# jswu18/projected-langevin-sampling

Measured on AMD Instinct MI355X. Metric: Langevin steps/sec, higher is better.
Workload: dtype f64; 1 GPU; configs[1]: synthetic regression N=1e5 M=1024 J=8192 D=8, RBF/ARD, ONB + Gaussian/identity, fp64; N=100000, M=1024, M_k=1024, J=8192, J_per_gpu=8192, parallelism=J-sharded x1, no per-step collective

## Files before the change

projected-langevin-sampling_amd/csrc/plship.hip:

```cpp
#include <hip/hip_runtime.h>

#include <atomic>
#include <cmath>
#include <cstdarg>
#include <cstdio>
#include <cstdlib>
#include <string>
#include <vector>

#define PLS_SCALAR_POLY_CONSTANTS 1
#include "../../include/plship.h"
#include "chol.h"
#include "common.h"
#include "cost_device.h"
#include "gemm_api.h"
#include "gemm_tn_f64.h"
#include "gemm_launch.h"
#include "gemm_tn_f64_kg.h"
#include "gemm_tn_f64_rows.h"
#include "cost_epilogues.h"
#include "philox.h"
#include "small_rank.h"
#include "small_rank_launch.h"
#include "small_rank_step.h"
// ... 2039 lines not shown

static int validate_onb(const pls_onb_desc *b) {
  PLS_REQUIRE(b != nullptr, "onb descriptor is NULL");
  PLS_REQUIRE(b->mk > 0 && b->n > 0, "onb: mk and n must be positive");
  PLS_REQUIRE(b->A && b->At && b->lam, "onb: A, At and lam must be set");
  PLS_REQUIRE(b->lda >= b->n && b->ldat >= b->mk, "onb: leading dimension too small");
  if (b->B) PLS_REQUIRE(b->ldb >= b->mk && b->c, "onb: B needs ldb >= mk and c");
  return PLS_OK;
}

int pls_onb_build_projection(const double *Vs, int64_t ldvs, const double *Kzx, int64_t ldkzx, int64_t m, int64_t mk,
                             int64_t n, double *A, int64_t lda, double *At, int64_t ldat, void *stream) {
  PLS_REQUIRE(Vs && Kzx && A && At, "onb_build_projection: NULL pointer");
  PLS_REQUIRE(m > 0 && mk > 0 && n > 0 && mk <= m, "onb_build_projection: bad sizes");
  PLS_REQUIRE(ldvs >= mk && ldkzx >= n && lda >= n && ldat >= mk, "onb_build_projection: leading dimension too small");
  int rc = pls_gemm_tn(Vs, ldvs, Kzx, ldkzx, A, lda, mk, n, m, 1.0, 0.0, stream);
  if (rc) return rc;
  return pls_gemm_tn(Kzx, ldkzx, Vs, ldvs, At, ldat, n, mk, m, 1.0, 0.0, stream);
}

int pls_onb_build_gaussian(const pls_onb_desc *basis, const double *y, double *B, int64_t ldb, double *c, void *stream) {
  int rc = validate_onb(basis);
  if (rc) return rc;
  PLS_REQUIRE(y && B && c && ldb >= basis->mk, "onb_build_gaussian: bad arguments");
  rc = pls_gemm_tn(basis->At, basis->ldat, basis->At, basis->ldat, B, ldb, basis->mk, basis->mk, basis->n, 1.0, 0.0, stream);
  if (rc) return rc;
  hipLaunchKernelGGL(matvec_rows_kernel, dim3((unsigned)basis->mk), dim3(256), 0, S(stream), basis->A, basis->lda,
                     basis->n, y, c);
  rc = check_launch("matvec_rows");
  if (rc) return rc;
  hipLaunchKernelGGL(matvec_rows_kernel, dim3(1), dim3(256), 0, S(stream), y, basis->n, basis->n, y, c + basis->mk);
  return check_launch("matvec_rows");
}

int pls_onb_forward(const pls_onb_desc *basis, const double *U, int64_t ldu, int64_t j, double *F, int64_t ldf,
                    void *stream) {
  int rc = validate_onb(basis);
  if (rc) return rc;
  PLS_REQUIRE(U && F && j >= 0 && ldu >= j && ldf >= j, "onb_forward: bad arguments");
  return pls_gemm_tn(basis->A, basis->lda, U, ldu, F, ldf, basis->n, j, basis->mk, 1.0, 0.0, stream);
}

int pls_onb_particle_update(const pls_onb_desc *basis, const double *U, int64_t ldu, const double *G, int64_t ldg,
                            int64_t j, double eta, const pls_noise_desc *noise, double *dU, int64_t lddu, void *stream) {
  int rc = validate_onb(basis);
  if (rc) return rc;
  rc = validate_noise(noise, j);
  if (rc) return rc;
  PLS_REQUIRE(U && G && dU && j >= 0 && ldu >= j && ldg >= j && lddu >= j, "onb_particle_update: bad arguments");
  PLS_REQUIRE(eta >= 0.0, "onb_particle_update: step size must be >= 0");
  if (j == 0) return PLS_OK;
  rc = pls_gemm_tn(basis->At, basis->ldat, G, ldg, dU, lddu, basis->mk, j, basis->n, 1.0, 0.0, stream);
  if (rc) return rc;
  hipLaunchKernelGGL(langevin_update_kernel, dim3((unsigned)cdiv(j, 256), rows_grid(cdiv(basis->mk, 8) * 4)), dim3(256), 0,
                     S(stream), dU, lddu, U, ldu, dU, lddu, 1, (int64_t)0, U, ldu, basis->lam, 0.0, basis->mk, j,
                     make_etap(eta, nullptr), 0, make_noisep(noise));
  return check_launch("langevin_update");
}


struct StepCall {
  const pls_cost_desc *cost;
  const double *y;
  const double *U;
  int64_t ldu, j;
  double eta;
  const pls_block_desc *blocks;
  const pls_noise_desc *noise;
  double *out;
  int64_t ldo;
  int32_t out_mode;
  double *energy_in;
  void *workspace;
  size_t workspace_bytes;
  hipStream_t st;
  EtaP etap() const { return make_etap(eta, blocks); }
  NoiseP noisep() const { return make_noisep(noise, blocks); }
  double *energy_sums() const { return blocks ? blocks->energy_sums : nullptr; }
  uint32_t *energy_sync() const { return blocks ? blocks->energy_sync : nullptr; }
};

static int validate_blocks(const pls_block_desc *b) {
  if (!b) return PLS_OK;
  PLS_REQUIRE(b->block_cols > 0 && b->eta != nullptr, "step_blocks: block_cols must be > 0 and eta set");
  return PLS_OK;
}

static int validate_step(const char *who, const StepCall &c, bool lagged) {
  if (int rc = validate_cost(c.cost)) return rc;
  if (int rc = validate_noise(c.noise, c.j)) return rc;
  if (int rc = validate_blocks(c.blocks)) return rc;
  if (lagged) return validate_lag(c.blocks);
  PLS_REQUIRE(!c.blocks || (!c.blocks->energy_partials && !c.blocks->energy_partials_prev && !c.blocks->energy_flush),
              "%s: lagged energies (energy_partials) exist on the Gaussian/identity routes only", who);
  return PLS_OK;
}

static int validate_step_call(const char *who, const StepCall &c, bool needs_y) {
  PLS_REQUIRE(c.U && c.out && (c.y || !needs_y), "%s: NULL pointer", who);
  PLS_REQUIRE(c.out != c.U, "%s: out must not alias the particles (ping-pong the particle buffers)", who);
  PLS_REQUIRE(c.j >= 0 && c.ldu >= c.j && c.ldo >= c.j, "%s: bad sizes", who);
  PLS_REQUIRE(c.eta >= 0.0, "%s: step size must be >= 0", who);
  PLS_REQUIRE(c.out_mode == 0 || c.out_mode == 1, "%s: out_mode must be 0 (delta) or 1 (new state)", who);
  return PLS_OK;
}

enum class StepRoute { Whitened, Fast, OneLaunch, General, Winograd };

static bool gaussian_fast_path(const double *B, const double *c, const pls_cost_desc *cost, int force_generic) {
  return !force_generic && B && c && cost->cost == PLS_COST_GAUSSIAN && cost->link == PLS_LINK_IDENTITY;
}

static bool ws_holds(size_t total, const void *workspace, size_t workspace_bytes) {
  return total == 0 || (workspace && total <= workspace_bytes);
}

static bool launch_bound(int64_t n, int64_t mk, int64_t j) { return j <= 4096 && 4.0 * (double)n * (double)mk * (double)j <= 8e9; }

static bool sr_step_route_for(const double *Lb, int64_t ldlb, int64_t mk, int64_t n, const double *y, int64_t j) {
  const int64_t mode = g_small_rank_step.load();
  if (mode == 0 || !small_rank_ok(Lb, ldlb, mk)) return false;
  if (reinterpret_cast<uintptr_t>(y) & 15) return false;
  return mode >= 2 || launch_bound(n, mk, j);
}

struct SrStepOperands {
  const double *Lb;
  int64_t ldlb, mk, n;
  const double *Vf;
  int64_t ldvf;
  const double *Uadd;
  int64_t lduadd;
  const double *lam;
  double pconst;
  int64_t n_data = -1;
};

static SrStepLayout sr_step_plan(int lead, int64_t mk, int64_t n, const StepCall &c) {
  return sr_step_layout(lead, mk, n, c.j, c.blocks && c.energy_in && c.blocks->energy_sums, c.blocks && c.blocks->step_sync);
}

static int sr_step_launch(const SrStepOperands &basis, const SrStepLayout &L, const StepCall &c, const NoiseP &nz) {
  char *w = static_cast<char *>(c.workspace);
  uint32_t *sync = c.blocks ? c.blocks->step_sync : nullptr;
  if (L.counters) {
    sync = reinterpret_cast<uint32_t *>(w + L.sync_off);
    hipError_t e = hipMemsetAsync(sync, 0, L.sync_bytes, c.st);
    if (e != hipSuccess) return fail(PLS_ERR_HIP, "onb_step: hipMemsetAsync: %s", hipGetErrorString(e));
  }
  const int64_t ncb = cdiv(c.j, 16);
  SrStepP p{};
  p.Lb = basis.Lb;
  p.ldlb = basis.ldlb;
  p.U = basis.Vf;
  p.ldu = basis.ldvf;
  p.Uadd = basis.Uadd;
  p.lduadd = basis.lduadd;
  p.y = c.y;
  p.lam = basis.lam;
  p.pconst = basis.pconst;
  p.N = basis.n;
  p.Ndata = basis.n_data >= 0 ? basis.n_data : basis.n;
  p.J = c.j;
  p.K = (int)basis.mk;
  p.rows_per_split = L.rows;
  p.nsplit = (int)L.ns;
  p.cp = make_costp(c.cost);
  p.out = c.out;
  p.ldo = c.ldo;
  p.add_u = c.out_mode;
  p.etap = c.etap();
  p.nz = nz;
  p.cb_sync = sync;
  p.chunk_sync = sync ? sync + ncb : nullptr;
  p.slab = reinterpret_cast<double *>(w + L.slab_off);
  p.vslab = p.slab ? p.slab + ncb * L.ns * basis.mk * 16 : nullptr;
  p.e = c.energy_in;
  p.esums = (c.blocks && c.energy_in) ? c.blocks->energy_sums : nullptr;
  p.sums16 = (c.blocks && c.energy_in) ? c.blocks->energy_sums16 : nullptr;
#ifdef PLS_SRS_PROBE
  p.debug_stop = getenv("PLS_SRS_STOP") ? atoi(getenv("PLS_SRS_STOP")) : 0;
#endif
  if (p.Ndata < p.N) return c.energy_in ? launch_small_rank_step_prior_value(p, c.st) : launch_small_rank_step_prior(p, c.st);
  return c.energy_in ? launch_small_rank_step_value(p, c.st) : launch_small_rank_step(p, c.st);
}

static int finish_energy_sums(const pls_block_desc *blocks, const double *energy_in, int64_t j, hipStream_t st) {
  if (!blocks || !energy_in) return PLS_OK;
  if (blocks->energy_sums) {
    hipLaunchKernelGGL(chunk_sums_kernel, dim3((unsigned)cdiv(j, 256)), dim3(256), 0, st, energy_in, j, blocks->energy_sums);
    if (int rc = check_launch("chunk_sums")) return rc;
  }
  if (blocks->energy_sums16) {
    hipLaunchKernelGGL(sums16_kernel, dim3((unsigned)cdiv(cdiv(j, 16), 256)), dim3(256), 0, st, energy_in, j, blocks->energy_sums16);
    if (int rc = check_launch("sums16")) return rc;
  }
  return PLS_OK;
}

static int finish_sums16(const pls_block_desc *blocks, const double *energy_in, int64_t j, hipStream_t st) {
  if (!blocks || !energy_in || !blocks->energy_sums16 || blocks->energy_partials) return PLS_OK;
  hipLaunchKernelGGL(sums16_kernel, dim3((unsigned)cdiv(cdiv(j, 16), 256)), dim3(256), 0, st, energy_in, j, blocks->energy_sums16);
  return check_launch("sums16");
}

static int fast_step(const FastOp &op, const StepCall &c, const char *who) {
  const int rc = fast_step_launch(op, c.U, c.ldu, c.j, c.etap(), c.noisep(), c.out, c.ldo, c.out_mode, c.energy_in, c.workspace,
                                  c.workspace_bytes, c.st, who, c.energy_sums(), c.energy_sync(), make_lag(c.blocks));
  return rc ? rc : finish_sums16(c.blocks, c.energy_in, c.j, c.st);
}


static FastOp onb_fast_op(const pls_onb_desc *b, const pls_cost_desc *c) {
  return FastOp{b->B, b->ldb, b->c, b->lam, b->mk, 1.0 / c->p[0], 0.5 / c->p[0], b->c + b->mk};
}

static bool wino_basis_ok(const pls_onb_desc *b) {
  auto al = [](const void *p, int64_t ld) { return (reinterpret_cast<uintptr_t>(p) & 15) == 0 && (ld & 1) == 0; };
  return b->mk % 16 == 0 && b->mk >= 512 && b->n % 4 == 0 && b->n >= 16384 && al(b->A, b->lda) && al(b->At, b->ldat);
}

constexpr int64_t kWinoMinChunk = 8192;

static bool wino_route_for(const pls_onb_desc *b, const double *planes, size_t planes_bytes, const double *U, int64_t ldu,
                           int64_t j) {
  return g_winograd.load() != 0 && planes && (reinterpret_cast<uintptr_t>(planes) & 15) == 0 && wino_basis_ok(b) &&
         planes_bytes >= 4 * wino_left_plane_bytes(b->mk, b->n) && j % 128 == 0 && j >= 2048 &&
         (reinterpret_cast<uintptr_t>(U) & 15) == 0 && (ldu & 1) == 0;
}

size_t pls_onb_winograd_bytes(const pls_onb_desc *basis) {
  return (basis && validate_onb(basis) == PLS_OK && wino_basis_ok(basis)) ? 4 * wino_left_plane_bytes(basis->mk, basis->n) : 0;
}

int pls_onb_winograd_prepare(const pls_onb_desc *basis, double *planes, size_t planes_bytes, void *stream) {
  int rc = validate_onb(basis);
  if (rc) return rc;
  PLS_REQUIRE(wino_basis_ok(basis), "onb_winograd_prepare: the basis' shape or operands do not take the Winograd route");
  const size_t plane = wino_left_plane_bytes(basis->mk, basis->n);
  PLS_REQUIRE(planes && (reinterpret_cast<uintptr_t>(planes) & 15) == 0 && planes_bytes >= 4 * plane,
              "onb_winograd_prepare: planes must be 16-byte aligned and hold %zu bytes", 4 * plane);
  const int64_t mh = basis->mk / 2, nh = basis->n / 2;
  {
    LaunchScope scope(PLS_TAG_OTHER, S(stream));
    hipLaunchKernelGGL(winograd_left_kernel, dim3((unsigned)cdiv(mh, 256), (unsigned)(nh < 8192 ? nh : 8192)), dim3(256), 0,
                       S(stream), basis->At, basis->ldat, nh, mh, planes, (int64_t)(plane / sizeof(double)));
  }
  return check_launch("winograd_left");
}

size_t pls_onb_step_workspace_bytes(const pls_onb_desc *basis, int64_t j, int64_t n_chunk) {
  if (!basis || j <= 0) return 0;
  if (n_chunk <= 0 || n_chunk > basis->n) n_chunk = basis->n;
  const size_t general = drift_layout(0, basis->mk, basis->n, j, n_chunk).total;
  const size_t one_launch = sr_step_query_bytes(0, basis->mk, basis->n, j);
  return general > one_launch ? general : one_launch;
}

static int onb_general_step(const pls_onb_desc *basis, const StepCall &c) {
  const DriftLayout L = drift_plan(0, basis->mk, basis->n, c.j, c.workspace_bytes);
  if (!c.workspace || L.total > c.workspace_bytes)
    return fail(PLS_ERR_WORKSPACE_TOO_SMALL, "onb_step: workspace %zu bytes, need at least %zu", c.workspace_bytes,
                pls_onb_step_workspace_bytes(basis, c.j, 128));
  char *w = static_cast<char *>(c.workspace);
  double *D = reinterpret_cast<double *>(w + L.d_off);
  const int64_t slab_stride = (int64_t)(L.mj / sizeof(double));
  EnergySink sink;
  if (c.energy_in) {
    sink.partial = reinterpret_cast<double *>(w + L.part_off);
    sink.rows_cap = L.part_rows;
    sink.e = c.energy_in;
    sink.prior_kind = 1;
    sink.P = c.U;
    sink.ldp = c.ldu;
    sink.m = basis->mk;
    sink.lam = basis->lam;
  }
  int64_t nslab = 1;
  int rc = stream_drift(basis->A, basis->lda, basis->At, basis->ldat, basis->mk, basis->n, c.U, c.ldu, c.j, make_costp(c.cost),
                        c.y, D, c.j, L.slabs, slab_stride, &nslab, reinterpret_cast<double *>(w + L.g_off), L.n_chunk, c.st,
                        c.energy_in ? &sink : nullptr);
  if (rc) return rc;
  {
    LaunchScope scope(PLS_TAG_LANGEVIN_UPDATE, c.st);
    hipLaunchKernelGGL(langevin_update_kernel, dim3((unsigned)cdiv(c.j, 256), rows_grid(cdiv(basis->mk, 8) * 4)), dim3(256), 0,
                       c.st, c.out, c.ldo, c.U, c.ldu, D, c.j, (int)nslab, slab_stride, c.U, c.ldu, basis->lam, 0.0, basis->mk,
                       c.j, c.etap(), c.out_mode, c.noisep());
  }
  rc = check_launch("langevin_update");
  if (rc) return rc;
  return finish_energy_sums(c.blocks, c.energy_in, c.j, c.st);
}

static int onb_wino_step(const pls_onb_desc *basis, const StepCall &c, const WinoLayout &L, const double *S) {
  char *w = static_cast<char *>(c.workspace);
  double *P = reinterpret_cast<double *>(w + L.p_off);
  double *Q = reinterpret_cast<double *>(w + L.q_off);
  double *part = reinterpret_cast<double *>(w + L.part_off);
  const int64_t mh = L.mh, nh = L.nh, jh = L.jh, mk = basis->mk;
  const int64_t splane = (int64_t)(L.s_plane / sizeof(double)), pslab = (int64_t)(L.p_slab / sizeof(double));
  const int64_t qplane = (int64_t)(L.q_plane / sizeof(double));
  int rc = PLS_OK;
  int64_t kchunk = 0;
  const int64_t nslab = wino_split_k(mh, jh, L.n_chunk, &kchunk);
  const CostP cp = make_costp(c.cost);
  const double *At = basis->At;
  const int64_t ldat = basis->ldat;
  for (int64_t p0 = 0, ci = 0; p0 < nh; p0 += L.n_chunk, ++ci) {
    const int64_t rows = (nh - p0 < L.n_chunk) ? (nh - p0) : L.n_chunk;
    rc = launch_cost_deriv_paired(basis->A + p0, basis->lda, nh, c.U, c.ldu, jh, rows, mk, Q, qplane, c.y + p0, cp,
                                  c.energy_in ? part : nullptr, c.j, c.st);
    if (rc) return rc;
    if (c.energy_in) {
      LaunchScope scope(PLS_TAG_OTHER, c.st);
      hipLaunchKernelGGL(column_reduce_kernel, dim3((unsigned)cdiv(c.j, 256)), dim3(256), 0, c.st, part, c.j, cdiv(rows, 32), c.j,
                         c.energy_in, ci == 0 ? 0 : 1, p0 + L.n_chunk >= nh ? 1 : 0, c.U, c.ldu, mk, basis->lam, 0.0, 1.0,
                         (const double *)nullptr);
      if ((rc = check_launch("column_reduce"))) return rc;
    }
    const double *S1 = S + p0 * mh, *S2 = S1 + splane, *S3 = S2 + splane, *S4 = S3 + splane;
    const double *A11 = At + p0 * ldat, *A12 = At + (nh + p0) * ldat, *A22 = A12 + mh;
    WinoProducts t{{A11, A12, S4, A22, S1, S2, S3},
                   {ldat, ldat, mh, ldat, mh, mh, mh},
                   {Q + WQ_G11 * qplane, Q + WQ_G21 * qplane, Q + WQ_G22 * qplane, Q + WQ_T4 * qplane, Q + WQ_T1 * qplane,
                    Q + WQ_T2 * qplane, Q + WQ_T3 * qplane},
                   nslab * pslab};
    rc = launch_wino_products(t, mh, jh, rows, nslab > 1 ? kchunk : 0, P, pslab, ci == 0 ? 0.0 : 1.0, c.st);
    if (rc) return rc;
  }
  {
    LaunchScope scope(PLS_TAG_LANGEVIN_UPDATE, c.st);
    hipLaunchKernelGGL(langevin_update_wino_kernel, dim3((unsigned)cdiv(jh, 256), rows_grid(cdiv(mh, 8) * 4)), dim3(256), 0, c.st,
                       c.out, c.ldo, c.U, c.ldu, P, (int)nslab, pslab, basis->lam, mh, jh, c.etap(), c.out_mode, c.noisep());
  }
  rc = check_launch("langevin_update_wino");
  if (rc) return rc;
  return finish_energy_sums(c.blocks, c.energy_in, c.j, c.st);
}

static int onb_step_impl(const pls_onb_desc *basis, const StepCall &c, int32_t force_generic, const double *wg_planes = nullptr,
                         size_t wg_bytes = 0) {
  int rc = validate_onb(basis);
  if (!rc) rc = validate_step("onb_step", c, true);
  if (rc) return rc;
  const bool fast = gaussian_fast_path(basis->B, basis->c, c.cost, force_generic);
  if (c.blocks && c.blocks->energy_flush) {
    PLS_REQUIRE(fast, "onb_step: energy_flush is for the Gaussian/identity fast path");
    PLS_REQUIRE(c.U && c.j > 0 && c.ldu >= c.j, "onb_step: energy_flush needs the particle matrix of the step calls");
    return fast_step_launch(onb_fast_op(basis, c.cost), c.U, c.ldu, c.j, c.etap(), c.noisep(), nullptr, 0, 0, nullptr, nullptr, 0,
                            c.st, "onb_step", nullptr, nullptr, make_lag(c.blocks));
  }
  if ((rc = validate_step_call("onb_step", c, true))) return rc;
  if (c.j == 0) return PLS_OK;
  StepRoute route = StepRoute::General;
  SrStepLayout sl{};
  if (fast) {
    route = StepRoute::Fast;
  } else if (sr_step_route_for(basis->At, basis->ldat, basis->mk, basis->n, c.y, c.j)) {
    sl = sr_step_plan(0, basis->mk, basis->n, c);
    if (ws_holds(sl.total, c.workspace, c.workspace_bytes)) route = StepRoute::OneLaunch;
  }
  WinoLayout wl{};
  if (route == StepRoute::General && wino_route_for(basis, wg_planes, wg_bytes, c.U, c.ldu, c.j)) {
    wl = wino_plan(basis->mk, basis->n, c.j, c.workspace_bytes);
    const int64_t min_chunk = wl.nh < kWinoMinChunk ? wl.nh : kWinoMinChunk;
    if (c.workspace && wl.total <= c.workspace_bytes && wl.n_chunk >= min_chunk) route = StepRoute::Winograd;
  }
  PLS_REQUIRE(fast || !c.blocks || (!c.blocks->energy_partials && !c.blocks->energy_partials_prev),
              "onb_step: lagged energies (energy_partials) exist on the Gaussian/identity fast path only");
  switch (route) {
    case StepRoute::Fast:
      return fast_step(onb_fast_op(basis, c.cost), c, "onb_step");
    case StepRoute::OneLaunch:
      return sr_step_launch(SrStepOperands{basis->At, basis->ldat, basis->mk, basis->n, c.U, c.ldu, nullptr, 0, basis->lam, 0.0},
                            sl, c, c.noisep());
    case StepRoute::Winograd:
      return onb_wino_step(basis, c, wl, wg_planes);
    default:
      return onb_general_step(basis, c);
  }
}

int pls_onb_step(const pls_onb_desc *basis, const pls_cost_desc *cost, const double *y, double *U, int64_t ldu,
                 int64_t j, double eta, const pls_noise_desc *noise, double *out, int64_t ldo, int32_t out_mode,
                 int32_t force_generic, double *energy_in, void *workspace, size_t workspace_bytes, void *stream) {
  return onb_step_impl(basis, StepCall{cost, y, U, ldu, j, eta, nullptr, noise, out, ldo, out_mode, energy_in, workspace,
                                       workspace_bytes, S(stream)}, force_generic);
}

int pls_onb_step_wg(const pls_onb_desc *basis, const pls_cost_desc *cost, const double *y, double *U, int64_t ldu, int64_t j,
                    double eta, const pls_noise_desc *noise, double *out, int64_t ldo, int32_t out_mode, int32_t force_generic,
                    const double *wg_planes, size_t wg_bytes, double *energy_in, void *workspace, size_t workspace_bytes,
                    void *stream) {
  return onb_step_impl(basis, StepCall{cost, y, U, ldu, j, eta, nullptr, noise, out, ldo, out_mode, energy_in, workspace,
                                       workspace_bytes, S(stream)}, force_generic, wg_planes, wg_bytes);
}

int pls_onb_step_blocks_wg(const pls_onb_desc *basis, const pls_cost_desc *cost, const double *y, double *U, int64_t ldu,
                           int64_t j, const pls_block_desc *blocks, const pls_noise_desc *noise, double *out, int64_t ldo,
                           int32_t out_mode, int32_t force_generic, const double *wg_planes, size_t wg_bytes, double *energy_in,
                           void *workspace, size_t workspace_bytes, void *stream) {
  PLS_REQUIRE(blocks != nullptr, "onb_step_blocks: block descriptor is NULL");
  return onb_step_impl(basis, StepCall{cost, y, U, ldu, j, 0.0, blocks, noise, out, ldo, out_mode, energy_in, workspace,
                                       workspace_bytes, S(stream)}, force_generic, wg_planes, wg_bytes);
}

int pls_onb_step_blocks(const pls_onb_desc *basis, const pls_cost_desc *cost, const double *y, double *U, int64_t ldu,
                        int64_t j, const pls_block_desc *blocks, const pls_noise_desc *noise, double *out, int64_t ldo,
                        int32_t out_mode, int32_t force_generic, double *energy_in, void *workspace,
                        size_t workspace_bytes, void *stream) {
  PLS_REQUIRE(blocks != nullptr, "onb_step_blocks: block descriptor is NULL");
  return onb_step_impl(basis, StepCall{cost, y, U, ldu, j, 0.0, blocks, noise, out, ldo, out_mode, energy_in, workspace,
                                       workspace_bytes, S(stream)}, force_generic);
}


size_t pls_onb_energy_workspace_bytes(const pls_onb_desc *basis, int64_t j, int64_t n_chunk) {
  if (!basis || j <= 0) return 0;
  if (n_chunk <= 0 || n_chunk > basis->n) n_chunk = basis->n;
  return energy_layout(0, basis->mk, j, n_chunk).total;
}

int pls_onb_energy(const pls_onb_desc *basis, const pls_cost_desc *cost, const double *y, const double *U, int64_t ldu,
                   int64_t j, double *e, int32_t force_generic, void *workspace, size_t workspace_bytes, void *stream) {
  int rc = validate_onb(basis);
  if (rc) return rc;
  rc = validate_cost(cost);
  if (rc) return rc;
  PLS_REQUIRE(U && e && y && j >= 0 && ldu >= j, "onb_energy: bad arguments");
  if (j == 0) return PLS_OK;
  if (gaussian_fast_path(basis->B, basis->c, cost, force_generic))
    return fast_energy_launch(onb_fast_op(basis, cost), U, ldu, j, e, workspace, workspace_bytes, S(stream), "onb_energy");
  const EnergyLayout L = energy_plan(0, basis->mk, basis->n, j, workspace_bytes);
  if (!workspace || L.part_rows < 2)
    return fail(PLS_ERR_WORKSPACE_TOO_SMALL, "onb_energy: workspace %zu bytes too small", workspace_bytes);
  return stream_cost(basis->A, basis->lda, basis->At, basis->ldat, basis->mk, basis->n, U, ldu, j, make_costp(cost), y,
                     reinterpret_cast<double *>(static_cast<char *>(workspace) + L.part_off), L.part_rows, L.n_chunk, e, 1, U,
                     ldu, basis->mk, basis->lam, 0.0, S(stream));
}

int pls_onb_prior_energy(const pls_onb_desc *basis, const double *U, int64_t ldu, int64_t j, const double *cost,
                         double *e, void *stream) {
  int rc = validate_onb(basis);
  if (rc) return rc;
  PLS_REQUIRE(U && e && j >= 0 && ldu >= j, "onb_prior_energy: bad arguments");
  if (j == 0) return PLS_OK;
  hipLaunchKernelGGL(column_reduce_kernel, dim3((unsigned)cdiv(j, 256)), dim3(256), 0, S(stream), cost, j,
                     (int64_t)(cost ? 1 : 0), j, e, 0, 1, U, ldu, basis->mk, basis->lam, 0.0, 1.0, (const double *)nullptr);
  return check_launch("column_reduce");
}


static int validate_ipb(const pls_ipb_desc *b) {
  PLS_REQUIRE(b != nullptr, "ipb descriptor is NULL");
  PLS_REQUIRE(b->m > 0 && b->n > 0, "ipb: m and n must be positive");
  PLS_REQUIRE(b->Kzx && b->Kxz, "ipb: Kzx and Kxz must be set");
  PLS_REQUIRE((b->Sf && b->Sb) || b->W || (b->Linv && b->LinvT),
              "ipb: k(Z,Z) must enter as substitution operators Sf / Sb (pls_chol_factor), as the inverse factor Linv / LinvT or as W");
  PLS_REQUIRE((b->Linv == nullptr) == (b->LinvT == nullptr), "ipb: Linv and LinvT go together");
  if (b->Linv) PLS_REQUIRE(b->ldlinv >= b->m && b->ldlinvt >= b->m, "ipb: ldlinv / ldlinvt < m");
  if (b->Q) PLS_REQUIRE(b->ldq >= b->m && b->ct, "ipb: Q needs ldq >= m and ct");
  PLS_REQUIRE((b->Sf == nullptr) == (b->Sb == nullptr), "ipb: Sf and Sb go together");
  PLS_REQUIRE(b->ldkzx >= b->n && b->ldkxz >= b->m, "ipb: leading dimension too small");
  if (b->W) PLS_REQUIRE(b->ldw >= b->m, "ipb: ldw < m");
  if (b->Sf) PLS_REQUIRE(b->ldsf >= b->m && b->ldsb >= b->m, "ipb: ldsf / ldsb < m");
  if (b->LcT) PLS_REQUIRE(b->ldlct >= b->m, "ipb: ldlct < m");
  if (b->B) PLS_REQUIRE(b->ldb >= b->m && b->c, "ipb: fast-path constants need ldb >= m and c");
  return PLS_OK;
}

static pls_chol_desc ipb_factor(const pls_ipb_desc *b) {
  return pls_chol_desc{b->m, nullptr, 0, b->LcT, b->ldlct, b->Sf, b->ldsf, b->Sb, b->ldsb, b->Linv, b->ldlinv, b->LinvT, b->ldlinvt,
                       b->tri_scratch, b->tri_scratch_bytes};
}

static int ipb_apply_kinv(const pls_ipb_desc *b, const double *U, int64_t ldu, int64_t j, double *V, void *stream,
                          double *tmp = nullptr) {
  const bool explicit_inverse = (!b->Sf && !b->Linv) || (g_ipb_explicit_inverse.load() != 0 && b->W);
  if (explicit_inverse) return pls_gemm_tn(b->W, b->ldw, U, ldu, V, j, b->m, j, b->m, 1.0, 0.0, stream);
  const pls_chol_desc f = ipb_factor(b);
  return chol_full_solve(&f, U, ldu, j, V, j, tmp, S(stream));
}

static bool ipb_whitened_ok(const pls_ipb_desc *b, const pls_cost_desc *c) {
  return b->Q && b->ct && b->LcT && b->ldq >= b->m && b->q_inv_noise == 1.0 / c->p[0] && (b->LinvT || (b->Sf && b->Sb)) &&
         g_ipb_explicit_inverse.load() == 0;
}

static FastOp ipb_whitened_op(const pls_ipb_desc *b) {
  return FastOp{b->Q, b->ldq, b->ct, nullptr, b->m, 1.0, 0.5 * b->q_inv_noise, b->ct + b->m};
}

int pls_ipb_forward(const pls_ipb_desc *basis, const double *U, int64_t ldu, int64_t j, double *F, int64_t ldf,
                    void *workspace, size_t workspace_bytes, void *stream) {
  int rc = validate_ipb(basis);
  if (rc) return rc;
  PLS_REQUIRE(U && F && j >= 0 && ldu >= j && ldf >= j, "ipb_forward: bad arguments");
  if (j == 0) return PLS_OK;
  const size_t need = (size_t)basis->m * j * sizeof(double);
  if (!workspace || workspace_bytes < need)
    return fail(PLS_ERR_WORKSPACE_TOO_SMALL, "ipb_forward: workspace %zu < %zu bytes", workspace_bytes, need);
  double *V = static_cast<double *>(workspace);
  rc = ipb_apply_kinv(basis, U, ldu, j, V, stream);
  if (rc) return rc;
  return pls_gemm_tn(basis->Kzx, basis->ldkzx, V, j, F, ldf, basis->n, j, basis->m, 1.0, 0.0, stream);
}

static int ipb_colour_noise(const pls_ipb_desc *basis, NoiseP &nz, int64_t j, double *xi_buf, double *e_buf, hipStream_t st) {
  if (nz.kind != PLS_NOISE_PHILOX) return PLS_OK;
  if (!basis->LcT) return fail(PLS_ERR_INVALID_ARGUMENT, "ipb: Philox noise needs the Cholesky factor LcT");
  hipLaunchKernelGGL(normal_fill_kernel, dim3((unsigned)cdiv(j, 256), rows_grid(cdiv(basis->m, 8) * 4)), dim3(256), 0, st,
                     xi_buf, j, basis->m, j, nz.seed, nz.step, nz.j_offset, nz.step_base, nz.block_cols);
  int rc = check_launch("normal_fill");
  if (rc) return rc;
  rc = gemm_tn_ex(basis->LcT, basis->ldlct, xi_buf, j, e_buf, j, basis->m, j, basis->m, 1.0, 0.0, 1, st, basis->tri_scratch,
                  basis->tri_scratch_bytes);
  if (rc) return rc;
  nz.kind = PLS_NOISE_INJECTED;
  nz.xi = e_buf;
  nz.ldxi = j;
  return PLS_OK;
}

static int ipb_finish(const pls_ipb_desc *basis, const double *U, int64_t ldu, const double *D, int nslab,
                      int64_t slab_stride, const double *V, int64_t j, double eta, const pls_noise_desc *noise, double *out, int64_t ldo, int add_u,
                      double *xi_buf, double *e_buf, hipStream_t st, const double *dsub = nullptr, double dsub_scale = 0.0,
                      const pls_block_desc *blocks = nullptr) {
  NoiseP nz = make_noisep(noise, blocks);
  if (int rc = ipb_colour_noise(basis, nz, j, xi_buf, e_buf, st)) return rc;
  hipLaunchKernelGGL(langevin_update_kernel, dim3((unsigned)cdiv(j, 256), rows_grid(cdiv(basis->m, 8) * 4)), dim3(256), 0, st,
                     out, ldo, U, ldu, D, j, nslab, slab_stride, V, j, (const double *)nullptr, (double)basis->m, basis->m, j,
                     make_etap(eta, blocks), add_u, nz, dsub, dsub_scale);
  return check_launch("langevin_update");
}

int pls_ipb_build_gaussian(const pls_ipb_desc *basis, const double *y, double *B, int64_t ldb, double *c, void *stream) {
  int rc = validate_ipb(basis);
  if (rc) return rc;
  PLS_REQUIRE(y && B && c && ldb >= basis->m, "ipb_build_gaussian: bad arguments");
  rc = pls_gemm_tn(basis->Kxz, basis->ldkxz, basis->Kxz, basis->ldkxz, B, ldb, basis->m, basis->m, basis->n, 1.0, 0.0, stream);
  if (rc) return rc;
  hipLaunchKernelGGL(matvec_rows_kernel, dim3((unsigned)basis->m), dim3(256), 0, S(stream), basis->Kzx, basis->ldkzx,
                     basis->n, y, c);
  rc = check_launch("matvec_rows");
  if (rc) return rc;
  hipLaunchKernelGGL(matvec_rows_kernel, dim3(1), dim3(256), 0, S(stream), y, basis->n, basis->n, y, c + basis->m);
  return check_launch("matvec_rows");
}

int pls_ipb_particle_update(const pls_ipb_desc *basis, const double *U, int64_t ldu, const double *G, int64_t ldg,
                            int64_t j, double eta, const pls_noise_desc *noise, double *dU, int64_t lddu,
                            void *workspace, size_t workspace_bytes, void *stream) {
  int rc = validate_ipb(basis);
  if (rc) return rc;
  rc = validate_noise(noise, j);
  if (rc) return rc;
  PLS_REQUIRE(U && G && dU && j >= 0 && ldu >= j && ldg >= j && lddu >= j, "ipb_particle_update: bad arguments");
  PLS_REQUIRE(eta >= 0.0, "ipb_particle_update: step size must be >= 0");
  if (j == 0) return PLS_OK;
  const size_t mj = align_up((size_t)basis->m * j * sizeof(double), 256);
  if (!workspace || workspace_bytes < 4 * mj)
    return fail(PLS_ERR_WORKSPACE_TOO_SMALL, "ipb_particle_update: workspace %zu < %zu bytes", workspace_bytes, 4 * mj);
  char *w = static_cast<char *>(workspace);
  double *V = reinterpret_cast<double *>(w), *D = reinterpret_cast<double *>(w + mj);
  double *xi = reinterpret_cast<double *>(w + 2 * mj), *e = reinterpret_cast<double *>(w + 3 * mj);
  rc = ipb_apply_kinv(basis, U, ldu, j, V, stream, xi);
  if (rc) return rc;
  rc = pls_gemm_tn(basis->Kxz, basis->ldkxz, G, ldg, D, j, basis->m, j, basis->n, 1.0, 0.0, stream);
  if (rc) return rc;
  return ipb_finish(basis, U, ldu, D, 1, (int64_t)0, V, j, eta, noise, dU, lddu, 0, xi, e, S(stream));
}

constexpr int IPB_LEAD = 3;

size_t pls_ipb_step_workspace_bytes(const pls_ipb_desc *basis, int64_t j, int64_t n_chunk) {
  if (!basis || j <= 0) return 0;
  if (n_chunk <= 0 || n_chunk > basis->n) n_chunk = basis->n;
  const size_t general = drift_layout(IPB_LEAD, basis->m, basis->n, j, n_chunk).total;
  const size_t one_launch = sr_step_query_bytes(IPB_LEAD, basis->m, basis->n, j);
  return general > one_launch ? general : one_launch;
}

static int ipb_whitened_route(const pls_ipb_desc *basis, const StepCall &c, const DriftLayout &L) {
  char *w = static_cast<char *>(c.workspace);
  double *Sw = reinterpret_cast<double *>(w), *Wd = reinterpret_cast<double *>(w + L.mj);
  double *epart = reinterpret_cast<double *>(w + 2 * L.mj);
  NoiseP nz = c.noisep();
  const bool injected = nz.kind == PLS_NOISE_INJECTED;
  const double *e_inj = injected ? nz.xi : nullptr;
  const int64_t ld_inj = nz.ldxi;
  if (injected) nz.kind = PLS_NOISE_NONE;
  int rc;
  if (basis->Pt && !c.energy_in && g_ipb_step_operator.load() != 0) {
    FastOp op = ipb_whitened_op(basis);
    op.B = basis->Pt;
    op.ldb = basis->ldpt;
    rc = fast_step_launch(op, c.U, c.ldu, c.j, c.etap(), nz, Wd, c.j, 0, nullptr, nullptr, 0, c.st, "ipb_step");
  } else {
    const pls_chol_desc f = ipb_factor(basis);
    rc = chol_forward_solve(&f, c.U, c.ldu, c.j, Sw, c.j, c.st);
    if (rc) return rc;
    rc = fast_step_launch(ipb_whitened_op(basis), Sw, c.j, c.j, c.etap(), nz, Wd, c.j, 0, c.energy_in, epart, 2 * L.mj, c.st,
                          "ipb_step", c.energy_sums(), c.energy_sync());
  }
  if (rc) return rc;
  rc = finish_sums16(c.blocks, c.energy_in, c.j, c.st);
  if (rc) return rc;
  EpiIpbFinish fin{c.out, c.ldo, c.U, c.ldu, c.out_mode, c.etap(), e_inj, ld_inj};
  return launch_gemm_any(basis->LcT, basis->ldlct, Wd, c.j, basis->m, c.j, basis->m, fin, c.st, 0, 1,
                         TriScratch{basis->tri_scratch, basis->tri_scratch_bytes});
}

static int ipb_fast_route(const pls_ipb_desc *basis, const StepCall &c, const DriftLayout &L) {
  char *w = static_cast<char *>(c.workspace);
  double *V = reinterpret_cast<double *>(w), *xi = reinterpret_cast<double *>(w + L.mj);
  double *e = reinterpret_cast<double *>(w + 2 * L.mj), *D = reinterpret_cast<double *>(w + L.d_off);
  int rc = ipb_apply_kinv(basis, c.U, c.ldu, c.j, V, c.st, xi);
  if (rc) return rc;
  const double inv_noise = 1.0 / c.cost->p[0];
// ... 404 lines not shown
```

projected-langevin-sampling_amd/csrc/step_plan.h:

```cpp
#pragma once
#include <cmath>
#include <cstddef>
#include <cstdint>
#ifdef PLS_SRS_PROBE
#include <cstdlib>
#endif

#include "common.h"
#include "small_rank.h"
#include "small_rank_step.h"

namespace plship {

static inline size_t mj_bytes(int64_t m, int64_t j) { return align_up((size_t)m * j * sizeof(double), 256); }

static inline int64_t plan_split_k(int64_t I, int64_t J, int64_t K, int64_t *kchunk) {
  const int64_t tiles = cdiv(I, 128) * cdiv(J, 128);
  int64_t s = 1;
  if (tiles < 512) s = cdiv(512, tiles);
  const int64_t s_local = cdiv(K, 16384);
  if (s_local > s) s = s_local;
  if (s > 16) s = 16;
  if (s > 1) {
    auto waste = [&](int64_t sl) {
      const double rounds = (double)(tiles * sl) / 512.0;
      return std::ceil(rounds) / rounds;
    };
    int64_t best = s;
    for (int64_t sl = s + 1; sl <= 16 && sl <= s + 4; ++sl)
      if (waste(sl) < waste(best) - 0.03) best = sl;
    s = best;
  }
  const int64_t min_chunk = tiles < 64 ? 256 : 1024;
  while (s > 1 && K / s < min_chunk) --s;
  int64_t kc = cdiv(cdiv(K, s), 16) * 16;
  s = cdiv(K, kc);
  *kchunk = (s > 1) ? kc : 0;
  return s;
}

static inline int64_t onb_max_slabs(int64_t mk, int64_t j, int64_t n) {
  int64_t kc;
  int64_t s = plan_split_k(mk, j, n, &kc);
  if (mk <= 256) {
    int64_t rows;
    const int64_t sr = small_rank_splits(j, n, &rows);
    if (sr > s) s = sr;
  }
  return s;
}

static inline int64_t energy_partial_rows(int64_t n_chunk) { return cdiv(n_chunk, 32) < 32 ? 32 : cdiv(n_chunk, 32); }
static inline size_t onb_energy_partial_bytes(int64_t n_chunk, int64_t j) {
  return align_up((size_t)energy_partial_rows(n_chunk) * j * sizeof(double), 256);
}

static inline int64_t gaussian_partial_rows(int64_t mk, bool big_tiles, bool step) {
  return big_tiles ? (step ? 2 : 1) * cdiv(mk, 128) : cdiv(mk, 64);
}
static inline size_t gaussian_partial_bytes(int64_t rows, int64_t j) { return (size_t)rows * j * sizeof(double); }
static inline size_t gaussian_step_partial_bytes(int64_t mk, int64_t j) { return gaussian_partial_bytes(gaussian_partial_rows(mk, true, true), j); }

struct SrStepLayout {
  int64_t ns, rows;
  size_t slab_off, slab_bytes;
  bool counters;
  size_t sync_off, sync_bytes;
  size_t total;
};

static inline SrStepLayout sr_step_layout(int lead, int64_t mk, int64_t n, int64_t j, bool sums, bool own_sync) {
  SrStepLayout L{};
  L.ns = small_rank_step_splits(j, n, (int)mk, &L.rows);
#ifdef PLS_SRS_PROBE
  if (const char *f = getenv("PLS_SRS_FORCE_NS")) {
    L.ns = atoi(f);
    L.rows = (cdiv(n, L.ns) + 63) / 64 * 64;
    L.ns = cdiv(n, L.rows);
  }
#endif
  L.slab_off = (size_t)lead * mj_bytes(mk, j);
  L.slab_bytes = L.ns > 1 ? align_up((size_t)cdiv(j, 16) * L.ns * ((size_t)mk + 1) * 16 * sizeof(double), 256) : 0;
  L.counters = (L.ns > 1 || sums) && !own_sync;
  L.sync_off = L.slab_off + L.slab_bytes;
  L.sync_bytes = small_rank_step_sync_words(j) * sizeof(uint32_t);
  L.total = L.sync_off + (L.counters ? align_up(L.sync_bytes, 256) : 0);
  return L;
}

static inline size_t sr_step_query_bytes(int lead, int64_t mk, int64_t n, int64_t j) {
  return (mk < 1 || mk > 128) ? 0 : sr_step_layout(lead, mk, n, j, true, false).total;
}

struct DriftLayout {
  size_t mj;
  int64_t slabs;
  int64_t n_chunk, part_rows;
  size_t d_off, part_off, g_off, total;
};

static inline DriftLayout drift_chunk(DriftLayout L, int64_t j, int64_t n_chunk) {
  L.n_chunk = n_chunk;
  L.part_rows = energy_partial_rows(n_chunk);
  L.g_off = L.part_off + onb_energy_partial_bytes(n_chunk, j);
  L.total = L.g_off + (size_t)n_chunk * j * sizeof(double);
  return L;
}

static inline DriftLayout drift_layout(int lead, int64_t mk, int64_t n, int64_t j, int64_t n_chunk) {
  DriftLayout L{};
  L.mj = mj_bytes(mk, j);
  L.slabs = onb_max_slabs(mk, j, n);
  L.d_off = (size_t)lead * L.mj;
  L.part_off = L.d_off + (size_t)L.slabs * L.mj;
  return drift_chunk(L, j, n_chunk);
}

static inline DriftLayout drift_plan(int lead, int64_t mk, int64_t n, int64_t j, size_t avail) {
  const DriftLayout all = drift_layout(lead, mk, n, j, n);
  if (all.total <= avail) return all;
  auto fits = [&](int64_t c) { return drift_chunk(all, j, c).total <= avail; };
  const int64_t min_rows = n < 128 ? n : 128;
  if (!fits(min_rows)) return drift_chunk(all, j, min_rows);
  const size_t left = avail - all.part_off;
  const double per_row = (double)j * sizeof(double) * (1.0 + 1.0 / 32.0);
  int64_t c = (int64_t)(((double)left - 32.0 * j * sizeof(double) - 512.0) / per_row);
  if (c > n) c = n;
  c = c / 128 * 128;
  while (c > min_rows && !fits(c)) c -= 128;
  while (c + 128 <= n && fits(c + 128)) c += 128;
  return drift_chunk(all, j, c < min_rows ? min_rows : c);
}

struct WinoLayout {
  int64_t mh, nh, jh;
  int64_t slabs;
  int64_t n_chunk, part_rows;
  size_t s_plane, p_slab, q_plane;
  size_t p_off, part_off, q_off, total;
};

static inline int64_t wino_split_k(int64_t mh, int64_t jh, int64_t K, int64_t *kchunk) {
  const int64_t tiles = 7 * cdiv(mh, 128) * cdiv(jh, 128);
  int64_t s = tiles < 512 ? cdiv(512, tiles) : 1;
  const int64_t s_local = cdiv(K, 16384);
  if (s_local > s) s = s_local;
  if (s > 16) s = 16;
  auto waste = [&](int64_t sl) {
    const double rounds = (double)(tiles * sl) / 512.0;
    return std::ceil(rounds) / rounds;
  };
  int64_t best = s;
  for (int64_t sl = s + 1; sl <= 16 && sl <= s + 4; ++sl)
    if (waste(sl) < waste(best) - 0.03) best = sl;
  s = best;
  while (s > 1 && K / s < 1024) --s;
  int64_t kc = cdiv(cdiv(K, s), 16) * 16;
  s = cdiv(K, kc);
  *kchunk = (s > 1) ? kc : 0;
  return s;
}

static inline size_t wino_left_plane_bytes(int64_t mk, int64_t n) { return align_up((size_t)(n / 2) * (mk / 2) * sizeof(double), 256); }

static inline WinoLayout wino_chunk(WinoLayout L, int64_t n_chunk) {
  L.n_chunk = n_chunk;
  L.part_rows = energy_partial_rows(n_chunk);
  L.q_plane = align_up((size_t)n_chunk * L.jh * sizeof(double), 256);
  L.q_off = L.part_off + align_up((size_t)L.part_rows * 2 * L.jh * sizeof(double), 256);
  L.total = L.q_off + 7 * L.q_plane;
  return L;
}

static inline WinoLayout wino_layout(int64_t mk, int64_t n, int64_t j, int64_t n_chunk) {
  WinoLayout L{};
  L.mh = mk / 2;
  L.nh = n / 2;
  L.jh = j / 2;
  int64_t kc;
  L.slabs = wino_split_k(L.mh, L.jh, n_chunk < L.nh ? n_chunk : L.nh, &kc);
  L.s_plane = wino_left_plane_bytes(mk, n);
  L.p_slab = align_up((size_t)L.mh * L.jh * sizeof(double), 256);
  L.p_off = 0;
  L.part_off = L.p_off + 7 * (size_t)L.slabs * L.p_slab;
  return wino_chunk(L, n_chunk);
}

static inline WinoLayout wino_plan(int64_t mk, int64_t n, int64_t j, size_t avail) {
  const int64_t nh = n / 2;
  const WinoLayout all = wino_layout(mk, n, j, nh);
  if (all.total <= avail) return all;
  const int64_t min_rows = nh < 128 ? nh : 128;
  int64_t c = nh / 128 * 128;
  while (c > min_rows && wino_layout(mk, n, j, c).total > avail) c -= 128;
  return wino_layout(mk, n, j, c < min_rows ? min_rows : c);
}

struct EnergyLayout {
  size_t part_off;
  int64_t part_rows;
  int64_t n_chunk;
  size_t gauss_bytes;
  size_t total;
};

static inline EnergyLayout energy_layout(int lead, int64_t mk, int64_t j, int64_t n_chunk) {
  EnergyLayout L{};
  L.part_off = (size_t)lead * mj_bytes(mk, j);
  L.n_chunk = n_chunk;
  L.part_rows = cdiv(n_chunk, 64) < 2 ? 2 : cdiv(n_chunk, 64);
  L.gauss_bytes = lead ? L.part_off + mj_bytes(mk, j) : gaussian_partial_bytes(gaussian_partial_rows(mk, false, false), j);
  const size_t generic = L.part_off + (size_t)L.part_rows * j * sizeof(double);
  L.total = generic > L.gauss_bytes ? generic : L.gauss_bytes;
  return L;
}

static inline EnergyLayout energy_plan(int lead, int64_t mk, int64_t n, int64_t j, size_t avail) {
  EnergyLayout L = energy_layout(lead, mk, j, 0);
  L.part_rows = avail > L.part_off ? (int64_t)((avail - L.part_off) / ((size_t)j * sizeof(double))) : 0;
  L.n_chunk = L.part_rows * 64 > n ? n : L.part_rows * 64 / 128 * 128;
  L.total = L.part_off + (size_t)L.part_rows * j * sizeof(double);
  return L;
}

}
```

projected-langevin-sampling_amd/csrc/winograd.h:

```cpp
#pragma once
#include "cost_device.h"
#include "gemm_tn_f64.h"

namespace plship {

enum WinoPlane { WQ_G11 = 0, WQ_G21 = 1, WQ_G22 = 2, WQ_T1 = 3, WQ_T2 = 4, WQ_T3 = 5, WQ_T4 = 6, kWinoPlanes = 7 };

template <int TI, int TJ>
__device__ __forceinline__ void winograd_store(const AccFrag<TI, TJ> &acc, double *Q, int64_t ldq, int64_t plane, int64_t prow0,
                                               int64_t pcol0, int lane, int64_t I, int64_t J) {
  static_assert(TI == 4 && TJ == 4, "paired 64 x 64 wave blocks");
  const int q = lane >> 4, c16 = lane & 15;
#pragma unroll
  for (int ta = 0; ta < 2; ++ta)
#pragma unroll
    for (int r = 0; r < 4; ++r) {
      const int64_t prow = prow0 + 16 * ta + 4 * r + q;
#pragma unroll
      for (int tb = 0; tb < 2; ++tb) {
        const int64_t pcol = pcol0 + 16 * tb + c16;
        const double g11 = acc.v[ta][tb][r], g12 = acc.v[ta][tb + 2][r];
        const double g21 = acc.v[ta + 2][tb][r], g22 = acc.v[ta + 2][tb + 2][r];
        const double t1 = g12 - g11, t2 = g22 - t1, t3 = g22 - g12, t4 = t2 - g21;
        if (prow < I && pcol < J) {
          double *o = Q + prow * ldq + pcol;
          o[WQ_G11 * plane] = g11;
          o[WQ_G21 * plane] = g21;
          o[WQ_G22 * plane] = g22;
          o[WQ_T1 * plane] = t1;
          o[WQ_T2 * plane] = t2;
          o[WQ_T3 * plane] = t3;
          o[WQ_T4 * plane] = t4;
        }
      }
    }
}

struct EpiWinoGauss {
  static constexpr int kTag = PLS_TAG_GEMM_COST_DERIV;
  double *Q;
  int64_t ldq, plane;
  const double *y;
  int64_t pair_i, pair_j;
  double inv_noise;
  double *vpart;
  int64_t ldp;
  __device__ void apply(AccFrag<4, 4> &acc, int64_t prow0, int64_t pcol0, int lane, int, int64_t I, int64_t J, double *) const {
    const int q = lane >> 4, c16 = lane & 15;
    double sq[4] = {0.0, 0.0, 0.0, 0.0};
#pragma unroll
    for (int ta = 0; ta < 4; ++ta)
#pragma unroll
      for (int r = 0; r < 4; ++r) {
        const int64_t prow = prow0 + 16 * (ta & 1) + 4 * r + q;
        const bool ok = prow < I;
        const double yv = ok ? -inv_noise * y[prow + (ta >> 1) * pair_i] : 0.0;
#pragma unroll
        for (int tb = 0; tb < 4; ++tb) {
          const double g = fma(acc.v[ta][tb][r], inv_noise, yv);
          acc.v[ta][tb][r] = g;
          if (vpart && ok) sq[tb] = fma(g, g, sq[tb]);
        }
      }
    if (vpart) {
      const double half_s2 = 0.5 / inv_noise;
#pragma unroll
      for (int tb = 0; tb < 4; ++tb) {
        double t = sq[tb];
        t += __shfl_xor(t, 16);
        t += __shfl_xor(t, 32);
        const int64_t pcol = pcol0 + 16 * (tb & 1) + c16;
        if (lane < 16 && prow0 < I && pcol < J) vpart[(prow0 / 32) * ldp + (tb >> 1) * pair_j + pcol] = t * half_s2;
      }
    }
    winograd_store<4, 4>(acc, Q, ldq, plane, prow0, pcol0, lane, I, J);
  }
};

template <int COST, int LINK>
struct EpiWinoCost {
  static constexpr int kTag = PLS_TAG_GEMM_COST_DERIV;
  double *Q;
  int64_t ldq, plane;
  const double *y;
  int64_t pair_i, pair_j;
  CostP cp;
  double *vpart;
  int64_t ldp;
  __device__ void apply(AccFrag<4, 4> &acc, int64_t prow0, int64_t pcol0, int lane, int wave, int64_t I, int64_t J,
                        double *lds) const {
    constexpr int STRIDE = 64 + EPI_PAD;
    CostP cp = this->cp;
    if constexpr (COST >= 0) {
      cp.cost = COST;
      cp.link = LINK;
    }
    const int q = lane >> 4, c16 = lane & 15;
    double *w = lds + wave * 16 * STRIDE;
    const int64_t lrow = prow0 + 16 * ((lane >> 4) & 1) + (lane & 15);
    const double yl = lrow < I ? y[lrow + (lane >> 5) * pair_i] : 0.0;
    double s = 0.0;
    auto slab = [&](auto ta_tag, bool to_lds) {
      constexpr int ta = decltype(ta_tag)::value;
#pragma unroll
      for (int tb = 0; tb < 4; ++tb)
#pragma unroll
        for (int r = 0; r < 4; ++r) {
          double &x = w[(4 * r + q) * STRIDE + tb * 16 + c16];
          if (to_lds)
            x = acc.v[ta][tb][r];
          else
            acc.v[ta][tb][r] = x;
        }
    };
    auto pass = [&](int ta, bool to_lds) {
      switch (ta) {
        case 0: slab(std::integral_constant<int, 0>{}, to_lds); break;
        case 1: slab(std::integral_constant<int, 1>{}, to_lds); break;
        case 2: slab(std::integral_constant<int, 2>{}, to_lds); break;
        default: slab(std::integral_constant<int, 3>{}, to_lds); break;
      }
    };
#pragma unroll 1
    for (int ta = 0; ta < 4; ++ta) {
      pass(ta, true);
      __builtin_amdgcn_wave_barrier();
#pragma unroll 1
      for (int rr = 0; rr < 16; ++rr) {
        const double yv = __shfl(yl, ta * 16 + rr);
        double &x = w[rr * STRIDE + lane];
        const double f = x;
        x = cost_deriv(cp, yv, f);
        if (vpart && prow0 + 16 * (ta & 1) + rr < I) s += cost_value(cp, yv, f);
      }
      __builtin_amdgcn_wave_barrier();
      pass(ta, false);
    }
    if (vpart) {
      const int64_t pcol = pcol0 + 16 * ((lane >> 4) & 1) + c16;
      if (prow0 < I && pcol < J) vpart[(prow0 / 32) * ldp + (lane >> 5) * pair_j + pcol] = s;
    }
    winograd_store<4, 4>(acc, Q, ldq, plane, prow0, pcol0, lane, I, J);
  }
};

template <class Epi>
__global__ __launch_bounds__(256, 2) void gemm_paired_kernel(GemmShape g, Epi epi) {
  extern __shared__ __attribute__((aligned(16))) double lds[];
  int tile_i, tile_j;
  gemm_tile_coords(blockIdx.x, g.nti, g.ntj, tile_i, tile_j);
  const int64_t i0 = (int64_t)tile_i * 64, j0 = (int64_t)tile_j * 64;
  AccFrag<4, 4> acc;
#pragma unroll
  for (int a = 0; a < 4; ++a)
#pragma unroll
    for (int b = 0; b < 4; ++b) acc.v[a][b] = double4_t{0.0, 0.0, 0.0, 0.0};
  const int wave = threadIdx.x >> 6, lane = threadIdx.x & 63;
  const int wr = wave >> 1, wc = wave & 1;
  if (i0 + 64 > g.I || j0 + 64 > g.J)
    gemm_tn_mainloop<128, 128, 64, 64, 16, true, true, true, 4, 16, 4, 4, true>(g, i0, j0, lds, acc, wr * 64);
  else
    gemm_tn_mainloop<128, 128, 64, 64, 16, true, false, true, 4, 16, 4, 4, true>(g, i0, j0, lds, acc, wr * 64);
  epi.apply(acc, i0 + 32 * wr, j0 + 32 * wc, lane, wave, g.I, g.J, lds);
}

template <class Epi>
static int launch_gemm_paired(const double *Lf, int64_t ldlf, int64_t pair_i, const double *V, int64_t ldv, int64_t pair_j,
                              int64_t rows, int64_t K, const Epi &epi, hipStream_t st) {
  constexpr size_t lds_bytes = (size_t)2 * 16 * ((128 + 16) + (128 + 16)) * sizeof(double);
  auto kern = gemm_paired_kernel<Epi>;
  static std::atomic<uint64_t> lds_ready{0};
  if (int rc = ensure_dynamic_lds(reinterpret_cast<const void *>(kern), lds_bytes, lds_ready)) return rc;
  GemmShape g{Lf, ldlf, V, ldv, rows, pair_j, K, 0, 0, 0, 0};
  g.pair_i = pair_i;
  g.pair_j = pair_j;
  g.nti = (int)cdiv(rows, 64);
  g.ntj = (int)cdiv(pair_j, 64);
  const int64_t nwg = (int64_t)g.nti * g.ntj;
  if (nwg <= 0) return PLS_OK;
  if (nwg > 0x7fffffff) return fail(PLS_ERR_INVALID_ARGUMENT, "gemm_paired: too many tiles");
  {
    LaunchScope scope(Epi::kTag, st);
    hipLaunchKernelGGL(kern, dim3((unsigned)nwg), dim3(256), lds_bytes, st, g, epi);
  }
  return check_launch("gemm_paired");
}

int launch_cost_deriv_paired(const double *Lf, int64_t ldlf, int64_t pair_i, const double *V, int64_t ldv, int64_t pair_j,
                             int64_t rows, int64_t kdim, double *Q, int64_t plane, const double *y, const CostP &cp, double *vpart,
                             int64_t ldp, hipStream_t st);

}
```

Measured before the change: 23.39 steps/s.

## Balance Winograd row chunks and add direct buffer-store epilogue for interior tiles

Row chunks in the ONB Winograd step are now sized evenly, rounded to multiples of 128, and the split-K slab count is capped at the preallocated slab count. The paired GEMM epilogue gains a direct path for interior tiles that computes the Winograd combinations in registers and writes them with raw buffer stores, skipping the bounds-checked generic store. The Gaussian epilogue gets a specialized direct path that preloads y once and fuses the cost derivative as an FMA. These changes aim to cut tail imbalance from ragged chunks and to lower epilogue store overhead. They add extra template paths, which may raise register pressure, and rely on a kDirectMaxLd limit defined elsewhere.

```diff
diff --git a/projected-langevin-sampling_amd/csrc/plship.hip b/projected-langevin-sampling_amd/csrc/plship.hip
--- a/projected-langevin-sampling_amd/csrc/plship.hip
+++ b/projected-langevin-sampling_amd/csrc/plship.hip
@@ -2365,19 +2365,20 @@
   const int64_t qplane = (int64_t)(L.q_plane / sizeof(double));
   int rc = PLS_OK;
   int64_t kchunk = 0;
-  const int64_t nslab = wino_split_k(mh, jh, L.n_chunk, &kchunk);
+  const int64_t walk = wino_balanced_chunk(nh, L.n_chunk);
+  const int64_t nslab = wino_walk_split_k(mh, jh, walk, L.slabs, &kchunk);
   const CostP cp = make_costp(c.cost);
   const double *At = basis->At;
   const int64_t ldat = basis->ldat;
-  for (int64_t p0 = 0, ci = 0; p0 < nh; p0 += L.n_chunk, ++ci) {
-    const int64_t rows = (nh - p0 < L.n_chunk) ? (nh - p0) : L.n_chunk;
+  for (int64_t p0 = 0, ci = 0; p0 < nh; p0 += walk, ++ci) {
+    const int64_t rows = (nh - p0 < walk) ? (nh - p0) : walk;
     rc = launch_cost_deriv_paired(basis->A + p0, basis->lda, nh, c.U, c.ldu, jh, rows, mk, Q, qplane, c.y + p0, cp,
                                   c.energy_in ? part : nullptr, c.j, c.st);
     if (rc) return rc;
     if (c.energy_in) {
       LaunchScope scope(PLS_TAG_OTHER, c.st);
       hipLaunchKernelGGL(column_reduce_kernel, dim3((unsigned)cdiv(c.j, 256)), dim3(256), 0, c.st, part, c.j, cdiv(rows, 32), c.j,
-                         c.energy_in, ci == 0 ? 0 : 1, p0 + L.n_chunk >= nh ? 1 : 0, c.U, c.ldu, mk, basis->lam, 0.0, 1.0,
+                         c.energy_in, ci == 0 ? 0 : 1, p0 + walk >= nh ? 1 : 0, c.U, c.ldu, mk, basis->lam, 0.0, 1.0,
                          (const double *)nullptr);
       if ((rc = check_launch("column_reduce"))) return rc;
     }
diff --git a/projected-langevin-sampling_amd/csrc/step_plan.h b/projected-langevin-sampling_amd/csrc/step_plan.h
--- a/projected-langevin-sampling_amd/csrc/step_plan.h
+++ b/projected-langevin-sampling_amd/csrc/step_plan.h
@@ -196,6 +196,23 @@
   return wino_layout(mk, n, j, c < min_rows ? min_rows : c);
 }
 
+static inline int64_t wino_balanced_chunk(int64_t nh, int64_t cap) {
+  if (cap >= nh) return nh;
+  const int64_t c = cdiv(nh, cap);
+  const int64_t rows = cdiv(cdiv(nh, c), 128) * 128;
+  return rows < cap ? rows : cap;
+}
+
+static inline int64_t wino_walk_split_k(int64_t mh, int64_t jh, int64_t rows, int64_t max_slabs, int64_t *kchunk) {
+  int64_t s = wino_split_k(mh, jh, rows, kchunk);
+  if (s > max_slabs) {
+    const int64_t kc = cdiv(cdiv(rows, max_slabs), 16) * 16;
+    s = cdiv(rows, kc);
+    *kchunk = (s > 1) ? kc : 0;
+  }
+  return s;
+}
+
 struct EnergyLayout {
   size_t part_off;
   int64_t part_rows;
diff --git a/projected-langevin-sampling_amd/csrc/winograd.h b/projected-langevin-sampling_amd/csrc/winograd.h
--- a/projected-langevin-sampling_amd/csrc/winograd.h
+++ b/projected-langevin-sampling_amd/csrc/winograd.h
@@ -36,8 +36,45 @@
     }
 }
 
+template <class Val>
+__device__ __forceinline__ void winograd_store_direct(double *Q, int64_t ldq, int64_t plane, int64_t prow0, int64_t pcol0, int lane,
+                                                      Val &&val) {
+#if defined(__HIP_DEVICE_COMPILE__)
+  double *corner = Q + prow0 * ldq + pcol0;
+  const int voff = (int)(((int64_t)(lane >> 4) * ldq + (lane & 15)) * 8);
+  const int ld4 = (int)(ldq * 32);
+  auto put = [&](int k, double v, int soff) {
+    const __amdgpu_buffer_rsrc_t rs = __builtin_amdgcn_make_buffer_rsrc(corner + k * plane, 0, 0x7FFFFFF0, 0x00020000);
+    __builtin_amdgcn_raw_buffer_store_b64(__builtin_bit_cast(u32x2_t, v), rs, voff, soff, 0);
+  };
+#pragma unroll
+  for (int ta = 0; ta < 2; ++ta)
+#pragma unroll
+    for (int r = 0; r < 4; ++r)
+#pragma unroll
+      for (int tb = 0; tb < 2; ++tb) {
+        const int soff = (ta * 4 + r) * ld4 + tb * 128;
+        const double g11 = val(ta, tb, r), g12 = val(ta, tb + 2, r);
+        const double g21 = val(ta + 2, tb, r), g22 = val(ta + 2, tb + 2, r);
+        const double t1 = g12 - g11, t2 = g22 - t1, t3 = g22 - g12, t4 = t2 - g21;
+        put(WQ_G11, g11, soff);
+        put(WQ_G21, g21, soff);
+        put(WQ_G22, g22, soff);
+        put(WQ_T1, t1, soff);
+        put(WQ_T2, t2, soff);
+        put(WQ_T3, t3, soff);
+        put(WQ_T4, t4, soff);
+        __builtin_amdgcn_sched_barrier(0);
+      }
+#else
+  (void)Q, (void)ldq, (void)plane, (void)prow0, (void)pcol0, (void)lane, (void)val;
+#endif
+}
+
 struct EpiWinoGauss {
   static constexpr int kTag = PLS_TAG_GEMM_COST_DERIV;
+  static constexpr bool kOwnDirect = true;
+  __device__ bool direct_ready() const { return vpart == nullptr; }
   double *Q;
   int64_t ldq, plane;
   const double *y;
@@ -45,6 +82,25 @@
   double inv_noise;
   double *vpart;
   int64_t ldp;
+  __device__ __forceinline__ void apply_direct(const AccFrag<4, 4> &acc, int64_t prow0, int64_t pcol0, int lane) const {
+#if defined(__HIP_DEVICE_COMPILE__)
+    const int yoff = (lane >> 4) * 8;
+    double yv[4][4];
+#pragma unroll
+    for (int ta = 0; ta < 4; ++ta) {
+      const __amdgpu_buffer_rsrc_t ys =
+          __builtin_amdgcn_make_buffer_rsrc(const_cast<double *>(y + prow0 + (ta >> 1) * pair_i), 0, 0x7FFFFFF0, 0x00020000);
+#pragma unroll
+      for (int r = 0; r < 4; ++r)
+        yv[ta][r] =
+            -inv_noise * __builtin_bit_cast(double, __builtin_amdgcn_raw_buffer_load_b64(ys, yoff, (16 * (ta & 1) + 4 * r) * 8, 0));
+    }
+    winograd_store_direct(Q, ldq, plane, prow0, pcol0, lane,
+                          [&](int ta, int tb, int r) { return fma(acc.v[ta][tb][r], inv_noise, yv[ta][r]); });
+#else
+    (void)acc, (void)prow0, (void)pcol0, (void)lane;
+#endif
+  }
   __device__ void apply(AccFrag<4, 4> &acc, int64_t prow0, int64_t pcol0, int lane, int, int64_t I, int64_t J, double *) const {
     const int q = lane >> 4, c16 = lane & 15;
     double sq[4] = {0.0, 0.0, 0.0, 0.0};
@@ -80,6 +136,7 @@
 template <int COST, int LINK>
 struct EpiWinoCost {
   static constexpr int kTag = PLS_TAG_GEMM_COST_DERIV;
+  static constexpr bool kOwnDirect = false;
   double *Q;
   int64_t ldq, plane;
   const double *y;
@@ -87,7 +144,7 @@
   CostP cp;
   double *vpart;
   int64_t ldp;
-  __device__ void apply(AccFrag<4, 4> &acc, int64_t prow0, int64_t pcol0, int lane, int wave, int64_t I, int64_t J,
+  __device__ void apply(AccFrag<4, 4> &acc, int64_t prow0, int64_t pcol0, int lane, int wave, bool direct, int64_t I, int64_t J,
                         double *lds) const {
     constexpr int STRIDE = 64 + EPI_PAD;
     CostP cp = this->cp;
@@ -140,7 +197,10 @@
       const int64_t pcol = pcol0 + 16 * ((lane >> 4) & 1) + c16;
       if (prow0 < I && pcol < J) vpart[(prow0 / 32) * ldp + (lane >> 5) * pair_j + pcol] = s;
     }
-    winograd_store<4, 4>(acc, Q, ldq, plane, prow0, pcol0, lane, I, J);
+    if (direct)
+      winograd_store_direct(Q, ldq, plane, prow0, pcol0, lane, [&](int ta, int tb, int r) { return acc.v[ta][tb][r]; });
+    else
+      winograd_store<4, 4>(acc, Q, ldq, plane, prow0, pcol0, lane, I, J);
   }
 };
 
@@ -157,11 +217,25 @@
     for (int b = 0; b < 4; ++b) acc.v[a][b] = double4_t{0.0, 0.0, 0.0, 0.0};
   const int wave = threadIdx.x >> 6, lane = threadIdx.x & 63;
   const int wr = wave >> 1, wc = wave & 1;
-  if (i0 + 64 > g.I || j0 + 64 > g.J)
-    gemm_tn_mainloop<128, 128, 64, 64, 16, true, true, true, 4, 16, 4, 4, true>(g, i0, j0, lds, acc, wr * 64);
-  else
-    gemm_tn_mainloop<128, 128, 64, 64, 16, true, false, true, 4, 16, 4, 4, true>(g, i0, j0, lds, acc, wr * 64);
-  epi.apply(acc, i0 + 32 * wr, j0 + 32 * wc, lane, wave, g.I, g.J, lds);
+  const bool edge = i0 + 64 > g.I || j0 + 64 > g.J;
+  const bool direct = !edge && epi.ldq < kDirectMaxLd;
+  if constexpr (Epi::kOwnDirect) {
+    if (direct && epi.direct_ready()) {
+      gemm_tn_mainloop<128, 128, 64, 64, 16, true, false, true, 4, 16, 4, 4, true>(g, i0, j0, lds, acc, wr * 64);
+      const int wu = __builtin_amdgcn_readfirstlane(wave);
+      epi.apply_direct(acc, i0 + 32 * (wu >> 1), j0 + 32 * (wu & 1), lane);
+    } else {
+      gemm_tn_mainloop<128, 128, 64, 64, 16, true, true, true, 4, 16, 4, 4, true>(g, i0, j0, lds, acc, wr * 64);
+      epi.apply(acc, i0 + 32 * wr, j0 + 32 * wc, lane, wave, g.I, g.J, lds);
+    }
+  } else {
+    if (edge)
+      gemm_tn_mainloop<128, 128, 64, 64, 16, true, true, true, 4, 16, 4, 4, true>(g, i0, j0, lds, acc, wr * 64);
+    else
+      gemm_tn_mainloop<128, 128, 64, 64, 16, true, false, true, 4, 16, 4, 4, true>(g, i0, j0, lds, acc, wr * 64);
+    const int wu = __builtin_amdgcn_readfirstlane(wave);
+    epi.apply(acc, i0 + 32 * (wu >> 1), j0 + 32 * (wu & 1), lane, wu, direct, g.I, g.J, lds);
+  }
 }
 
 template <class Epi>
```

After: 23.59 steps/s, median of 6. Within noise of the previous version (+0.9%).
